# agentmorris/MegaDetector

Hardware: AMD Instinct MI355X
Metric: images/sec (whole node) MDv5a @1280px batch inference (higher is better)
Workload: dtype bf16

## Files before the change

include/mdhip.h:

```cpp
#ifndef MDHIP_H
#define MDHIP_H

#include <stddef.h>
#include <stdint.h>

#include "mdjpeg.h"

#ifdef __cplusplus
extern "C" {
#endif

#define MDHIP_OK            0
#define MDHIP_EINVAL       -1
#define MDHIP_EHIP         -2
#define MDHIP_ENOMEM       -3
#define MDHIP_EUNSUPPORTED -4
#define MDHIP_ECAPACITY    -5

#define MDHIP_DTYPE_BF16 0
#define MDHIP_DTYPE_FP8  1
#define MDHIP_DTYPE_FP16 2

#define MDHIP_CONV      0
#define MDHIP_C3        1
// ... 198 lines not shown
int mdhip_read_op_tensor(mdhip_ctx* ctx, int op, int which, int n, float* out, int* c, int* h, int* w, void* hip_stream);
int mdhip_read_op_weights(mdhip_ctx* ctx, int op, float* w, float* b, int* c_out, int* c_in, int* kh, int* kw);

int mdhip_dwconv3x3_on(mdhip_ctx* ctx, const uint16_t* in, int ld_in, const float* weight, const float* bias, const uint16_t* res,
                       uint16_t* out, int n, int h, int w, int c, int grp, int grp_stride, int grp_off, int act, void* hip_stream);
int mdhip_attention_on(mdhip_ctx* ctx, const uint16_t* qkv, uint16_t* out, int n, int n_tokens, int heads, void* hip_stream);
int mdhip_dfl_decode_on(mdhip_ctx* ctx, const float* box, const float* cls, int nc, int n, int ny, int nx, float stride, float* pred,
                        void* hip_stream);

int mdhip_adown_pool_on(mdhip_ctx* ctx, const uint16_t* in, uint16_t* a, uint16_t* b, int n, int h, int w, int c_in,
                        void* hip_stream);
int mdhip_cbfuse_on(mdhip_ctx* ctx, const uint16_t* const* src, const int32_t* factor, int n_src, const uint16_t* last,
                    uint16_t* out, int n, int h, int w, int c, void* hip_stream);

typedef struct {
    char    name[48];
    int32_t kind;
    int32_t layer;
    int32_t m, n, k;
    double  flops;
    double  bytes;
    int32_t cfg;
    int32_t ntaps, stride, has_res;
} mdhip_op_info;

long long mdhip_plan_describe(const mdhip_model* model, int dtype, int max_batch, int max_h, int max_w, char* buf, size_t cap);
int mdhip_num_ops(mdhip_ctx* ctx);
int mdhip_get_op_info(mdhip_ctx* ctx, int op, mdhip_op_info* out);
int mdhip_forward_timed(mdhip_ctx* ctx, int n, int h, int w, float* ms, void* hip_stream);
int mdhip_time_forwards(mdhip_ctx* ctx, int enable);
int mdhip_forward_times(mdhip_ctx* ctx, float* ms, int max_n);
int mdhip_set_op_cfg(mdhip_ctx* ctx, int op, int cfg);
int mdhip_num_conv_cfgs(void);
int mdhip_op_supports_cfg(mdhip_ctx* ctx, int op, int cfg);
int mdhip_cfg_is_bitwise(int cfg);
const char* mdhip_conv_cfg_name(int cfg);
typedef struct {
    int32_t m, n, k;
    int32_t ntaps, stride;
    int32_t has_res;
    int32_t cfg;
    int32_t batch;
} mdhip_tuned;
int mdhip_set_tuned(mdhip_ctx* ctx, const mdhip_tuned* entries, int n);
int mdhip_set_fuse(mdhip_ctx* ctx, int on);
int mdhip_set_graph(mdhip_ctx* ctx, int mode, int max_n);
int mdhip_set_option(mdhip_ctx* ctx, const char* name, int value);
int mdhip_time_op(mdhip_ctx* ctx, int op, int n, int h, int w, int iters, float* ms_avg,
                  void* hip_stream);
#define MDHIP_LAUNCHES_NO_FUSE 1
#define MDHIP_LAUNCHES_NO_FUSE_DECODE 2
#define MDHIP_LAUNCHES_NO_PAIR 4
#define MDHIP_LAUNCHES_ISOLATED 8
#define MDHIP_LAUNCHES_CALIBRATING 16
#define MDHIP_LAUNCHES_AUGMENTED 32
#define MDHIP_LAUNCHES_AFTER_OTHERS 64
long long mdhip_launches_describe(const mdhip_model* model, int dtype, int max_batch, int max_h, int max_w, const mdhip_tuned* tuned,
                                  int n_tuned, int n, int h, int w, unsigned flags, const int32_t* forced, int n_forced, char* buf,
                                  size_t cap);

const char* mdhip_version(void);

#ifdef __cplusplus
}
#endif
#endif
```

megadetector_amd/_lib.py:

```python

import ctypes as C
import os

import numpy as np

from .jpeg_host import mdjpeg_change_options

_HERE = os.path.dirname(os.path.abspath(__file__))
LIB_PATH = os.path.join(_HERE, 'libmdhip.so')

MDHIP_OK = 0
MDHIP_EINVAL = -1
MDHIP_ECAPACITY = -5
MDHIP_EUNSUPPORTED = -4
MDHIP_DTYPE_BF16 = 0
MDHIP_DTYPE_FP8 = 1
MDHIP_DTYPE_FP16 = 2
MDHIP_LAUNCHES_NO_FUSE, MDHIP_LAUNCHES_NO_FUSE_DECODE, MDHIP_LAUNCHES_NO_PAIR, MDHIP_LAUNCHES_ISOLATED = 1, 2, 4, 8
MDHIP_LAUNCHES_CALIBRATING, MDHIP_LAUNCHES_AUGMENTED, MDHIP_LAUNCHES_AFTER_OTHERS = 16, 32, 64


class mdhip_conv(C.Structure):
    _fields_ = [('weight', C.POINTER(C.c_float)), ('bias', C.POINTER(C.c_float)),
                ('c_out', C.c_int32), ('c_in', C.c_int32), ('kh', C.c_int32), ('kw', C.c_int32)]


class mdhip_layer(C.Structure):
    _fields_ = [('type', C.c_int32), ('n_from', C.c_int32), ('from_', C.c_int32 * 4),
                ('c_out', C.c_int32), ('k', C.c_int32), ('s', C.c_int32), ('p', C.c_int32),
                ('n', C.c_int32), ('shortcut', C.c_int32), ('first_conv', C.c_int32)]


class mdhip_model(C.Structure):
    _fields_ = [('n_layers', C.c_int32), ('layers', C.POINTER(mdhip_layer)),
                ('n_convs', C.c_int32), ('convs', C.POINTER(mdhip_conv)),
                ('nc', C.c_int32), ('na', C.c_int32), ('nl', C.c_int32),
                ('anchors_px', C.POINTER(C.c_float)), ('strides', C.POINTER(C.c_float))]


class mdhip_letterbox(C.Structure):
    _fields_ = [('src_h', C.c_int32), ('src_w', C.c_int32), ('resized_h', C.c_int32),
                ('resized_w', C.c_int32), ('top', C.c_int32), ('left', C.c_int32), ('interp', C.c_int32)]
# ... 16 lines not shown
class mdhip_classifier_crop(C.Structure):
    _fields_ = [('src', C.c_void_p), ('pitch', C.c_int64), ('src_w', C.c_int32), ('src_h', C.c_int32),
                ('canvas_w', C.c_int32), ('canvas_h', C.c_int32), ('off_x', C.c_int32), ('off_y', C.c_int32)]


class mdhip_thumbnail(C.Structure):
    _fields_ = [('src', C.c_void_p), ('pitch', C.c_int64), ('src_w', C.c_int32), ('src_h', C.c_int32),
                ('canvas_w', C.c_int32), ('canvas_h', C.c_int32), ('off_x', C.c_int32), ('off_y', C.c_int32),
                ('out_w', C.c_int32), ('out_h', C.c_int32), ('dst', C.c_void_p), ('dst_pitch', C.c_int64)]


class mdhip_rde_box(C.Structure):
    _fields_ = [('x', C.c_double), ('y', C.c_double), ('w', C.c_double), ('h', C.c_double),
                ('group', C.c_int32), ('category', C.c_int32)]


mdhip_change_options = mdjpeg_change_options


class mdhip_op_info(C.Structure):
    _fields_ = [('name', C.c_char * 48), ('kind', C.c_int32), ('layer', C.c_int32),
                ('m', C.c_int32), ('n', C.c_int32), ('k', C.c_int32),
                ('flops', C.c_double), ('bytes', C.c_double), ('cfg', C.c_int32),
                ('ntaps', C.c_int32), ('stride', C.c_int32), ('has_res', C.c_int32)]


class mdhip_tuned(C.Structure):
    _fields_ = [('m', C.c_int32), ('n', C.c_int32), ('k', C.c_int32), ('ntaps', C.c_int32),
                ('stride', C.c_int32), ('has_res', C.c_int32), ('cfg', C.c_int32), ('batch', C.c_int32)]


_P = C.c_void_p
SYMBOLS = {
    'mdhip_create': (C.c_int, [C.POINTER(mdhip_model), C.c_int, C.c_int, C.c_int, C.c_int, C.c_int, C.POINTER(_P)]),
    'mdhip_create_images': (C.c_int, [C.c_int, C.POINTER(_P)]),
    'mdhip_destroy': (None, [_P]),
    'mdhip_last_error': (C.c_char_p, [_P]),
    'mdhip_preprocess': (C.c_int, [_P, C.POINTER(_P), C.POINTER(mdhip_letterbox), C.c_int, C.c_int, C.c_int, _P]),
    'mdhip_preprocess_windows': (C.c_int, [_P, C.POINTER(_P), C.POINTER(mdhip_letterbox), C.POINTER(C.c_int64),
                                           C.POINTER(C.c_int64), C.c_int, C.c_int, C.c_int, _P]),
    'mdhip_forward': (C.c_int, [_P, C.c_int, C.c_int, C.c_int, _P]),
    'mdhip_jpeg_reconstruct': (C.c_int, [_P, C.POINTER(mdhip_jpeg_image), C.c_int, C.POINTER(_P), _P]),
    'mdhip_jpeg_entropy_decode': (C.c_int, [_P, C.POINTER(mdhip_jpeg_scan), C.c_int, C.c_int, C.POINTER(C.c_int32), _P]),
    'mdhip_jpeg_entropy_stats': (C.c_int, [_P, C.POINTER(C.c_int64)]),
    'mdhip_jpeg_recompress': (C.c_int, [_P, C.POINTER(_P), C.POINTER(C.c_int32), C.POINTER(C.c_int32), C.POINTER(C.c_int64),
                                        C.c_int, C.POINTER(C.c_uint16), C.POINTER(C.c_uint16), C.POINTER(_P), _P]),
    'mdhip_jpeg_encode': (C.c_int, [_P, C.POINTER(_P), C.POINTER(C.c_int32), C.POINTER(C.c_int32), C.POINTER(C.c_int64), C.c_int,
# ... 109 lines not shown
```

megadetector_amd/csrc/conv_v2.cpp:

```cpp

#include <algorithm>
#include <type_traits>

#include "conv_device.h"

namespace mdhip {
namespace MDHIP_ST {

namespace {

constexpr int v2_lds_bytes(int bm, int bn) { return 2 * (bm + bn) * 128; }
constexpr int v2_ring_lds_bytes(int bm, int bn) { return (3 * bm + 2 * bn) * 128; }
constexpr int v2_blocks_per_cu(int bm, int bn, int nw) {
    int b = 163840 / v2_lds_bytes(bm, bn);
    if (b > 32 / nw) b = 32 / nw;
    if (b > 2) b = 2;
    return b < 1 ? 1 : b;
}
constexpr int v2_waves_per_simd(int bm, int bn, int nw) {
    int w = v2_blocks_per_cu(bm, bn, nw) * nw / 4;
    return w < 1 ? 1 : w;
}

}
// ... 459 lines not shown
        advance();
        if constexpr (RA == 3) {
            lb_advance();
            ca = ca == 2 ? 0 : ca + 1;
        }
        stamp(4);
        if (++c_kt == KT) {
            epilogue(c_tile);
            c_kt = 0;
            c_tile += tile_step;
        }
        stamp(5);
    }
    if constexpr ((PROF & 1) != 0) {
        if (lane == 0 && p.dbg) {
            unsigned long long* d = (unsigned long long*)p.dbg + ((size_t)blockIdx.x * NW + wave) * 8;
            for (int k = 0; k < 6; ++k) d[k] = t_acc[k];
            d[6] = (unsigned long long)total_steps;
            d[7] = (unsigned long long)__builtin_amdgcn_s_getreg(((4 - 1) << 11) | (0 << 6) | 20) ;
        }
    }
#endif
}

#define MDHIP_CONV2_CFGS(X) \
    X(0, 160, 160, 2, 2)    \
    X(1, 128, 160, 2, 2)    \
    X(2, 160, 80, 2, 1)     \
    X(3, 128, 80, 4, 1)     \
    X(4, 96, 160, 2, 2)     \
    X(5, 64, 160, 1, 2)     \
    X(6, 192, 160, 4, 2)    \
    X(7, 256, 160, 4, 2)    \
    X(8, 320, 160, 4, 2)
#define MDHIP_CONV2_RING(X) \
    X(9, 96, 160, 2, 2)     \
    X(10, 64, 160, 1, 2)    \
    X(11, 320, 160, 4, 2)   \
    X(12, 256, 160, 4, 2)
#define MDHIP_CONV2_DEC(X) \
    X(0, 160, 160, 2, 2)   \
    X(2, 160, 80, 2, 1)    \
    X(3, 128, 80, 4, 1)    \
    X(8, 320, 160, 4, 2)
#define MDHIP_CONV2_PROF(X) \
    X(13, 160, 160, 2, 2, 1)  \
// ... 13 lines not shown
    {bm, bn, (wm) * (wn) * 64, (size_t)v2_lds_bytes(bm, bn), v2_blocks_per_cu(bm, bn, (wm) * (wn)), \
     "v2:" #bm "x" #bn "/" #wm "x" #wn},
    MDHIP_CONV2_CFGS(X)
#undef X
#define X(id, bm, bn, wm, wn)                                                                        \
    {bm, bn, (wm) * (wn) * 64, (size_t)v2_ring_lds_bytes(bm, bn), 163840 / v2_ring_lds_bytes(bm, bn) >= 2 ? 2 : 1, "v2:" #bm "x" #bn "/" #wm "x" #wn "/a3"},
    MDHIP_CONV2_RING(X)
#undef X
#define X(id, bm, bn, wm, wn, prof)                                                                  \
    {bm, bn, (wm) * (wn) * 64, (size_t)v2_lds_bytes(bm, bn), v2_blocks_per_cu(bm, bn, (wm) * (wn)), \
     "v2prof" #prof ":" #bm "x" #bn "/" #wm "x" #wn},
    MDHIP_CONV2_PROF(X)
#undef X
#define X(id, bm, bn, wm, wn, prof)                                                                  \
    {bm, bn, (wm) * (wn) * 64, (size_t)v2_ring_lds_bytes(bm, bn), 1, "v2prof" #prof ":" #bm "x" #bn "/" #wm "x" #wn "/a3"},
    MDHIP_CONV2_PROFRING(X)
#undef X
};
constexpr int kNumPlain2 = 0 MDHIP_CONV2_CFGS(MDHIP_COUNT_ROW);
constexpr int kNumCfgs2 = kNumPlain2 MDHIP_CONV2_RING(MDHIP_COUNT_ROW);
constexpr int kNumProf = 0 MDHIP_CONV2_PROF(MDHIP_COUNT_ROW) MDHIP_CONV2_PROFRING(MDHIP_COUNT_ROW);

namespace {
enum { V2_PLAIN = 0, V2_PW1, V2_PW2, V2_UP, V2_DEV, V2_DEV_PW };
ConvInstTable conv2_insts() {
    static const ConvInst t[] = {
#define X(id, bm, bn, wm, wn)                                                                                         \
    MDHIP_INST(id, V2_PLAIN, (wm) * (wn) * 64, v2_lds_bytes(bm, bn), conv_v2_kernel<bm, bn, wm, wn>)                  \
    MDHIP_INST(id, V2_PW1, (wm) * (wn) * 64, v2_lds_bytes(bm, bn), conv_v2_kernel<bm, bn, wm, wn, 0, false, 1>)       \
    MDHIP_INST(id, V2_PW2, (wm) * (wn) * 64, v2_lds_bytes(bm, bn), conv_v2_kernel<bm, bn, wm, wn, 0, false, 2>)
        MDHIP_CONV2_CFGS(X)
#undef X
#define X(id, bm, bn, wm, wn)                                                                                         \
    MDHIP_INST(id, V2_PW1, (wm) * (wn) * 64, v2_ring_lds_bytes(bm, bn), conv_v2_kernel<bm, bn, wm, wn, 0, false, 1, 3>) \
    MDHIP_INST(id, V2_PW2, (wm) * (wn) * 64, v2_ring_lds_bytes(bm, bn), conv_v2_kernel<bm, bn, wm, wn, 0, false, 2, 3>)
        MDHIP_CONV2_RING(X)
#undef X
#define X(id, bm, bn, wm, wn, prof) MDHIP_INST(id, V2_DEV, (wm) * (wn) * 64, v2_lds_bytes(bm, bn), conv_v2_kernel<bm, bn, wm, wn, prof>)
        MDHIP_CONV2_PROF(X)
#undef X
#define X(id, bm, bn, wm, wn, prof) MDHIP_INST(id, V2_DEV_PW, (wm) * (wn) * 64, v2_ring_lds_bytes(bm, bn), conv_v2_kernel<bm, bn, wm, wn, prof, false, 1, 3>)
        MDHIP_CONV2_PROFRING(X)
#undef X
#define X(id, bm, bn, wm, wn) MDHIP_INST(id, CONV_KEY_DEC, (wm) * (wn) * 64, v2_lds_bytes(bm, bn), conv_v2_kernel<bm, bn, wm, wn, 0, false, 1, 2, 1>)
        MDHIP_CONV2_DEC(X)
#undef X
        MDHIP_INST(0, V2_UP, 256, v2_lds_bytes(160, 160), conv_v2_kernel<160, 160, 2, 2, 0, true>)
    };
    return {t, (int)(sizeof(t) / sizeof(t[0]))};
}
const ConvInst* conv2_pick(int cfg, const ConvArgs& a) {
    const ConvInstTable t = conv2_insts();
    if (a.in_up) return a.dec_pred ? nullptr : conv_find_inst(t, cfg, V2_UP);
    const bool pw = a.ntaps == 1 && a.stride == 1 && a.pad == 0 && a.H == a.Ho && a.W == a.Wo, whole = (a.C8 & 7) == 0;
    if (a.dec_pred) return pw && whole && a.out_f32 ? conv_find_inst(t, cfg, CONV_KEY_DEC) : nullptr;
    if (cfg >= kNumCfgs2) {
        const ConvInst* dev = conv_find_inst(t, cfg, V2_DEV);
        return dev || !(pw && whole) ? dev : conv_find_inst(t, cfg, V2_DEV_PW);
    }
    return conv_find_inst(t, cfg, !pw ? V2_PLAIN : whole ? V2_PW1 : V2_PW2);
}

bool conv2_cfg_is_ring(int cfg) { return cfg >= kNumPlain2 && cfg < kNumCfgs2; }
bool conv2_shape_ok(const ConvArgs& a) {
    if (a.in_up && !(a.ntaps == 1 && a.stride == 1 && (a.H % 2) == 0 && (a.W % 2) == 0 && a.up_slabs > 0 &&
                     a.up_slabs * 8 <= a.C8 && !a.in_f8))
        return false;
    return a.C8 >= 8 && a.kw <= 3 && a.ntaps <= 9 && (a.k_pad % 64) == 0;
}
bool conv2_supports(int cfg, const ConvArgs& a) {
    if (cfg < 0 || cfg >= kNumCfgs2 + kNumProf) return false;
    if (conv2_cfg_is_ring(cfg) && a.k_pad < 3 * 64) return false;
    return conv2_shape_ok(a) && conv2_pick(cfg, a) != nullptr;
}

hipError_t conv2_launch(int cfg, const ConvArgs& a, hipStream_t s) {
    if (cfg < 0 || cfg >= kNumCfgs2 + kNumProf || !conv2_shape_ok(a)) return hipErrorInvalidValue;
    ConvArgs p = a;
    conv_set_rcp(p);
    const dim3 grid = conv_tile_grid(p, g_cfgs2[cfg]);
    return conv_launch_inst(conv2_pick(cfg, a), grid, p, s);
}
}

MDHIP_CONV_FAMILY(conv_v2, CONV_V2, g_cfgs2, kNumCfgs2, kNumProf, true, false, true, conv2_supports, conv2_launch, conv2_insts)

}
}
```

megadetector_amd/csrc/mdhip_capi.cpp:

```cpp

#include <algorithm>
#include <climits>
#include <cmath>
#include <cstdarg>
#include <cstdio>
#include <cstdlib>
#include <cstring>

#include "mdhip_ctx.h"

static thread_local std::string g_create_error;

int mdhip::fail(mdhip_ctx* ctx, int code, const char* fmt, ...) {
    char buf[512];
    va_list ap;
    va_start(ap, fmt);
    vsnprintf(buf, sizeof(buf), fmt, ap);
    va_end(ap);
    if (ctx) ctx->err = buf; else g_create_error = buf;
    return code;
}

int mdhip::check_shape(mdhip_ctx* ctx, int n, int h, int w) {
    if (n < 1 || n > ctx->max_batch) return fail(ctx, MDHIP_EINVAL, "batch %d outside [1,%d]", n, ctx->max_batch);
// ... 213 lines not shown
    return (long long)text.size();
}

long long mdhip_launches_describe(const mdhip_model* model, int dtype, int max_batch, int max_h, int max_w, const mdhip_tuned* tuned,
                                  int n_tuned, int n, int h, int w, unsigned flags, const int32_t* forced, int n_forced, char* buf,
                                  size_t cap) {
    if (int rc = check_create_args(model, dtype, max_batch, max_h, max_w)) return rc;
    if (n_tuned < 0 || (n_tuned > 0 && !tuned) || n_forced < 0 || (n_forced > 0 && !forced))
        return fail(nullptr, MDHIP_EINVAL, "mdhip_launches_describe: bad table or forced list");
    mdhip_ctx ctx;
    ctx.pair_enabled = !(flags & MDHIP_LAUNCHES_NO_PAIR);
    PlannedWeights pw;
    std::string err;
    if (int rc = plan_context(&ctx, model, dtype, max_batch, max_h, max_w, &pw, &err)) return fail(nullptr, rc, "%s", err.c_str());
    ctx.arena = (char*)(uintptr_t)(1ull << 40);
    ctx.warena = (char*)(uintptr_t)(2ull << 40);
    int rc = check_shape(&ctx, n, h, w);
    if (!rc) rc = mdhip_set_tuned(&ctx, tuned, n_tuned);
    for (int i = 0; i < n_forced && !rc; ++i) rc = mdhip_set_op_cfg(&ctx, forced[2 * i], forced[2 * i + 1]);
    if (rc) return fail(nullptr, rc, "%s", ctx.err.empty() ? "mdhip_launches_describe: bad forced list" : ctx.err.c_str());
    const bool fuse = !(flags & MDHIP_LAUNCHES_NO_FUSE), fuse_decode = !(flags & MDHIP_LAUNCHES_NO_FUSE_DECODE);
    (void)mdhip_set_fuse(&ctx, fuse);
    (void)mdhip_set_option(&ctx, "fuse_decode", fuse_decode);
    auto resolve_as = [&](unsigned kind, int rn, int rh, int rw) {
        Pass pass(&ctx, nullptr, num_anchors_for(&ctx, rh, rw), (kind & MDHIP_LAUNCHES_ISOLATED) != 0, (kind & MDHIP_LAUNCHES_CALIBRATING) != 0);
        if (kind & MDHIP_LAUNCHES_AUGMENTED) ctx.cur_tta.scale = 0.83f;
        return resolved_for(&ctx, rn, rh, rw);
    };
    if (flags & MDHIP_LAUNCHES_AFTER_OTHERS)
        for (int round = 0; round < 4; ++round) {
            (void)mdhip_set_fuse(&ctx, round == 1 ? !fuse : fuse);
            (void)mdhip_set_option(&ctx, "fuse_decode", round == 2 ? !fuse_decode : fuse_decode);
            for (unsigned kind : {0u, (unsigned)MDHIP_LAUNCHES_ISOLATED, (unsigned)MDHIP_LAUNCHES_CALIBRATING, (unsigned)MDHIP_LAUNCHES_AUGMENTED}) {
                (void)resolve_as(kind, n, h, w);
                (void)resolve_as(kind, 1, ctx.max_stride * 2, ctx.max_stride * 3);
            }
        }
    const std::string text = describe_launches(&ctx, *resolve_as(flags, n, h, w));
    if (buf && cap) snprintf(buf, cap, "%s", text.c_str());
    return (long long)text.size();
}

void mdhip_destroy(mdhip_ctx* ctx) {
    if (!ctx) return;
    (void)hipSetDevice(ctx->device);
    drop_graphs(ctx);
// ... 516 lines not shown
                    w[(((size_t)oc * CI + ci) * KH + r) * KW + q] = st_to_f32(p[k], f16);
                }
    return MDHIP_OK;
}

int mdhip_num_ops(mdhip_ctx* ctx) { return ctx ? (int)ctx->ops.size() : MDHIP_EINVAL; }

int mdhip_get_op_info(mdhip_ctx* ctx, int op, mdhip_op_info* out) {
    NEED_MODEL(ctx);
    if (!ctx || !out || op < 0 || op >= (int)ctx->ops.size()) return MDHIP_EINVAL;
    const Op& o = ctx->ops[op];
    memset(out, 0, sizeof(*out));
    snprintf(out->name, sizeof(out->name), "%s", o.name.c_str());
    out->kind = o.kind == OP_DFL ? OP_DECODE : o.kind;
    if (o.kind == OP_ADOWN || o.kind == OP_CBFUSE) out->kind = o.kind - 1;
    out->layer = o.layer;
    const Launch L = ctx->last_ran ? ctx->last_ran->ops[op] : Launch();
    out->m = L.gm;
    out->n = L.gn;
    out->k = L.gk;
    out->flops = L.flops;
    out->bytes = L.bytes;
    out->cfg = L.how == RUN_IN_FRONT ? -2 : (o.kind == OP_CONV && L.how == RUN_LAUNCH) ? L.cfg : -1;
    if (o.kind == OP_CONV || o.kind == OP_DW) {
        const PackedConv& pc = ctx->packed[o.pc];
        out->ntaps = pc.kh * pc.kw;
        out->stride = o.stride;
        out->has_res = o.has_res ? 1 : 0;
    }
    return MDHIP_OK;
}

int mdhip_num_conv_cfgs(void) { return conv_num_cfgs(); }

int mdhip_op_supports_cfg(mdhip_ctx* ctx, int op, int cfg) {
    NEED_MODEL(ctx);
    if (!ctx || op < 0 || op >= (int)ctx->ops.size()) return MDHIP_EINVAL;
    if (ctx->ops[op].kind != OP_CONV || cfg < 0 || cfg >= conv_num_cfgs()) return 0;
    ConvArgs a{};
    const int h = ctx->last_h ? ctx->last_h : ctx->max_stride, w = ctx->last_w ? ctx->last_w : ctx->max_stride;
    conv_args(ctx, ctx->ops[op], ctx->last_n ? ctx->last_n : 1, h, w, a);
    return conv_api(ctx).supports(cfg, a) ? 1 : 0;
}

const char* mdhip_conv_cfg_name(int cfg) { return (cfg >= 0 && cfg < conv_num_cfgs()) ? conv_cfg(cfg).name : ""; }

// ... 2 lines not shown
int mdhip_set_tuned(mdhip_ctx* ctx, const mdhip_tuned* entries, int n) {
    NEED_MODEL(ctx);
    if (!ctx || n < 0 || (n > 0 && !entries)) return MDHIP_EINVAL;
    for (int i = 0; i < n; ++i)
        if (entries[i].cfg < 0 || entries[i].cfg >= conv_num_cfgs())
            return fail(ctx, MDHIP_EINVAL, "tuned entry %d: cfg %d outside [0,%d)", i, entries[i].cfg, conv_num_cfgs());
    ctx->tuned.assign(entries, entries + n);
    launches_changed(ctx);
    return MDHIP_OK;
}

int mdhip_set_fuse(mdhip_ctx* ctx, int on) {
    NEED_MODEL(ctx);
    ctx->fuse_enabled = on != 0;
    launches_changed(ctx);
    return MDHIP_OK;
}

int mdhip_set_option(mdhip_ctx* ctx, const char* name, int value) {
    NEED_MODEL(ctx);
    if (!ctx || !name) return MDHIP_EINVAL;
    if (!strcmp(name, "letterbox_general")) ctx->letterbox_general = value != 0;
    else if (!strcmp(name, "fuse_decode")) ctx->fuse_decode = value != 0;
    else return fail(ctx, MDHIP_EINVAL, "unknown option '%s'", name);
    launches_changed(ctx);
    return MDHIP_OK;
}

int mdhip_set_graph(mdhip_ctx* ctx, int mode, int max_n) {
    NEED_MODEL(ctx);
    if (!ctx || mode < 0 || mode > 2) return MDHIP_EINVAL;
    ctx->graph_mode = mode;
    if (max_n > 0) ctx->graph_max_n = max_n;
    if (mode == 0) drop_graphs(ctx);
    return MDHIP_OK;
}

int mdhip_set_op_cfg(mdhip_ctx* ctx, int op, int cfg) {
    NEED_MODEL(ctx);
    if (!ctx || op < 0 || op >= (int)ctx->ops.size()) return MDHIP_EINVAL;
    if (ctx->ops[op].kind != OP_CONV) return fail(ctx, MDHIP_EINVAL, "op %d is not a conv", op);
    if (cfg < -1 || cfg >= conv_num_cfgs()) return fail(ctx, MDHIP_EINVAL, "cfg %d outside [-1,%d)", cfg, conv_num_cfgs());
    ctx->ops[op].forced_cfg = cfg;
    launches_changed(ctx);
    return MDHIP_OK;
}
// ... 3 lines not shown
```

megadetector_amd/csrc/mdhip_ctx.h:

```cpp
#pragma once

#include <map>
#include <memory>
#include <string>
#include <tuple>
#include <vector>

#include "../../include/mdhip.h"
#include "mdhip_internal.h"

using namespace mdhip;

namespace mdhip {

int fail(mdhip_ctx* ctx, int code, const char* fmt, ...);

#define HIP_TRY(ctx, expr)                                                                   \
    do {                                                                                     \
        hipError_t e__ = (expr);                                                             \
        if (e__ != hipSuccess)                                                               \
            return fail(ctx, MDHIP_EHIP, "%s failed: %s (%s:%d)", #expr, hipGetErrorString(e__), \
                        __FILE__, __LINE__);                                                 \
    } while (0)

// ... 160 lines not shown
    NmsScratch nms_scr{};
    size_t nms_kv_off[6] = {}, nms_seg_off = 0;
    size_t nms_out_off = 0, nms_cnt_off = 0;
    size_t geom_off = 0;
    DevBuffer stage;
    DevBuffer jpeg_planes;
    DevBuffer jpeg_entropy;
    DevBuffer jpeg_encode;
    DevBuffer blur;
    DevBuffer resample;
    DevBuffer draw;
    DevBuffer classify;
    DevBuffer change;
    long long jpeg_entropy_stats[4] = {0, 0, 0, 0};
    int last_n = 0, last_h = 0, last_w = 0;
    int step_n = 0, step_h = 0, step_w = 0;
    std::string err;
    bool calibrated = false, calibrating = false;
    int n_f8 = 0;
    std::vector<std::vector<int>> fuse_groups;
    bool fuse_enabled = true, fuse_suspended = false;
    bool pair_enabled = true;
    bool fuse_decode = true;
    bool letterbox_general = false;
    std::vector<hipEvent_t> events;
    std::vector<mdhip_tuned> tuned;
    static constexpr int kFwdRing = 64;
    bool time_forward = false;
    hipEvent_t fwd_ev[kFwdRing][2] = {};
    long long fwd_count = 0;
    uint8_t* geom_host = nullptr;
    int geom_slot = 0;
    hipEvent_t geom_ev[4] = {nullptr, nullptr, nullptr, nullptr};
    float* nms_host_out[MDHIP_NMS_SLOTS] = {};
    int32_t* nms_host_cnt[MDHIP_NMS_SLOTS] = {};
    hipEvent_t nms_ev[MDHIP_NMS_SLOTS] = {};
    int nms_slot_n[MDHIP_NMS_SLOTS] = {};
    int graph_mode = 0;
    int graph_max_n = 8;
    hipStream_t capture_stream = nullptr;
    struct GraphSlot { hipGraphExec_t exec = nullptr; int seen = 0; bool disabled = false; long long last_use = 0; };
    std::map<std::tuple<int, int, int, int>, GraphSlot> graphs;
    static constexpr int kMaxGraphs = 32;
    long long graph_clock = 0;
    std::map<std::tuple<int, int, int, int>, std::shared_ptr<Resolved>> resolved;
    static constexpr int kMaxResolved = 64;
// ... 9 lines not shown
```

megadetector_amd/csrc/mdhip_exec.cpp:

```cpp

#include <algorithm>
#include <cmath>
#include <cstring>

#include "mdhip_ctx.h"

namespace mdhip {

const ConvRegistry& conv_api(const mdhip_ctx* ctx) { return ctx->dtype == MDHIP_DTYPE_FP16 ? st_f16::conv_registry : st_bf16::conv_registry; }
int conv_num_cfgs() { return st_bf16::conv_registry.num_cfgs(); }
const ConvCfg& conv_cfg(int i) { return st_bf16::conv_registry.cfg(i); }
bool conv_cfg_is_bitwise_family(int c) { return st_bf16::conv_registry.is_bitwise_family(c); }

int choose_cfg(int M, int n_rows) {
    const ConvFamily& v1 = *st_bf16::conv_registry.fam[CONV_IGEMM];
    int best = 0;
    float best_score = -1.f;
    for (int i = 0; i < v1.n_cfgs; ++i) {
        const ConvCfg& c = v1.cfgs[i];
        const int tn = (n_rows + c.bn - 1) / c.bn, tm = (M + c.bm - 1) / c.bm;
        const float useful = ((float)n_rows / (tn * c.bn)) * ((float)M / ((float)tm * c.bm));
        const float fill = std::min(1.0f, (float)tm * tn / 512.0f);
        const float score = useful * (0.35f + 0.65f * fill) * c.prior;
        if (score > best_score) { best_score = score; best = i; }
// ... 38 lines not shown
    a.k_pad = pc.k_pad;
    a.ntaps = pc.kh * pc.kw;
    a.kw = pc.kw;
    a.stride = op.stride;
    a.pad = op.pad;
    a.act = op.act;
    a.out_f32 = op.out_f32;
    if (op.out_f32) {
        a.out = ctx->arena + op.f32_off;
        a.ld_out = op.f32_ld;
    } else {
        a.out = ctx->arena + op.out.off;
        a.ld_out = op.out.ld;
    }
    a.res = op.has_res ? (const uint16_t*)(ctx->arena + op.res.off) : nullptr;
    a.ld_res = op.has_res ? op.res.ld : 0;
    a.tiles_n = 1;
    a.out_qscale = 1.0f;
    a.wgt4 = pc.w4_off ? (const uint16_t*)(ctx->warena + pc.w4_off) : nullptr;
    a.k_pad4 = pc.k_pad4;
    a.groups = pc.groups;
    a.wgt4p = (pc.w4p_off && ctx->pair_enabled) ? (const uint16_t*)(ctx->warena + pc.w4p_off) : nullptr;
    a.k_pad4p = pc.k_pad4p;
    if (ctx->dtype == MDHIP_DTYPE_FP8 && !ctx->calibrating) {
        if (op.f8_in) {
            a.in_f8 = 1;
            a.wgt8 = (const uint8_t*)(ctx->warena + pc.w8_off);
            a.scale = (const float*)(ctx->warena + pc.scale_off);
            a.k_pad8 = pc.k_pad8;
            a.groups8 = pc.groups8;
            a.C8 = (op.in.c + 15) / 16;
        }
        a.out_f8 = op.f8_out ? 1 : 0;
    }
}

namespace {

void conv_stats(const mdhip_ctx* ctx, const Op& op, const ConvArgs& a, int n, Launch& L) {
    const PackedConv& pc = ctx->packed[op.pc];
    L.gm = a.M;
    L.gn = pc.c_out;
    L.gk = pc.k_real;
    L.flops = 2.0 * (double)a.M * pc.c_out * pc.k_real;
    L.bytes = (double)n * a.H * a.W * op.in.c * 2.0 + (double)a.M * pc.c_out * (op.out_f32 ? 4.0 : 2.0) +
              (double)pc.c_out * pc.k_real * 2.0 + (op.has_res ? (double)a.M * pc.c_out * 2.0 : 0.0);
// ... 323 lines not shown
```

megadetector_amd/csrc/mdhip_internal.h:

```cpp
#pragma once

#include <hip/hip_runtime.h>
#include <stdint.h>

#include <algorithm>

struct MdClassifyCrop;

struct ChgWeights;
struct MdjImage;
struct MdjEncCrop;
struct MdjEncTables;
struct MdjKeepRect;

namespace mdhip {

__host__ __device__ inline uint16_t f32_to_bf16(float f) {
    union { float f; uint32_t u; } v;
    v.f = f;
    uint32_t u = v.u;
    if ((u & 0x7fffffffu) > 0x7f800000u) return (uint16_t)((u >> 16) | 0x40);
    u += 0x7fffu + ((u >> 16) & 1u);
    return (uint16_t)(u >> 16);
}
// ... 77 lines not shown
    int out_f32;
    int tiles_n, tiles_m, tiles_per_xcd, m_streams;
    const uint16_t* wgt4;
    int k_pad4, groups;
    const uint16_t* wgt4p;
    int k_pad4p;
    const uint8_t* wgt8;
    const float*   scale;
    int k_pad8, groups8;
    int in_f8, out_f8;
    float out_qscale;
    void* dbg;
    int dev_param;
    const uint16_t* wgt_pre;
    const float*    bias_pre;
    int k_pad_pre;
    const uint16_t* in_up;
    int ld_up, up_slabs;
    float* dec_pred;
    const float* dec_anchors;
    float dec_stride;
    int dec_level_off, dec_n_anchors;
    unsigned rcp_howo, rcp_wo;
};
inline unsigned conv_rcp32(int d) { return d <= 1 ? 0xffffffffu : (unsigned)(0x100000000ull / (unsigned)d); }
inline void conv_set_rcp(ConvArgs& p) { p.rcp_howo = conv_rcp32(p.HoWo); p.rcp_wo = conv_rcp32(p.Wo); }
#if defined(__HIP_DEVICE_COMPILE__) || defined(__HIPCC__)
__device__ __forceinline__ float mdhip_sigmoid_exact(float x) { return 1.0f / (1.0f + expf(-x)); }
__device__ __forceinline__ void mdhip_decode_box(float l0, float l1, float l2, float l3, int x, int y, float stride, float aw, float ah,
                                                 float& cx, float& cy, float& bw, float& bh) {
#pragma clang fp contract(off)
    const float s0 = mdhip_sigmoid_exact(l0), s1 = mdhip_sigmoid_exact(l1);
    const float s2 = mdhip_sigmoid_exact(l2), s3 = mdhip_sigmoid_exact(l3);
    cx = (s0 * 2.0f + ((float)x - 0.5f)) * stride;
    cy = (s1 * 2.0f + ((float)y - 0.5f)) * stride;
    const float w2 = s2 * 2.0f, h2 = s3 * 2.0f;
    bw = (w2 * w2) * aw;
    bh = (h2 * h2) * ah;
}
#endif

struct ConvCfg {
    int bm, bn, threads;
    size_t lds_bytes;
    int blocks_per_cu;
    const char* name;
// ... 21 lines not shown
constexpr int CONV_KEY_DEC = 100;
#define MDHIP_INST(local, key, threads, lds, ...) {(const void*)(__VA_ARGS__), (local), (key), (threads), (size_t)(lds)},
inline const ConvInst* conv_find_inst(ConvInstTable t, int local, int key) {
    for (int i = 0; i < t.n; ++i)
        if (t.rows[i].local == local && t.rows[i].key == key) return &t.rows[i];
    return nullptr;
}
inline hipError_t conv_launch_inst(const ConvInst* inst, dim3 grid, const ConvArgs& p, hipStream_t s) {
    if (!inst) return hipErrorInvalidValue;
    void* args[] = {(void*)&p};
    return hipLaunchKernel(inst->fn, grid, dim3((unsigned)inst->threads), args, inst->lds_bytes, s);
}

struct ConvFamily {
    ConvFamilyId id;
    const ConvCfg* cfgs;
    int n_cfgs, n_dev;
    bool bitwise;
    bool f8_in;
    bool f8_out;
    bool (*supports)(int local, const ConvArgs& a);
    hipError_t (*launch)(int local, const ConvArgs& a, hipStream_t s);
    ConvInstTable (*insts)();
};
#if defined(__HIP_DEVICE_COMPILE__)
#define MDHIP_CONV_FAMILY(name, ...)
#else
#define MDHIP_CONV_FAMILY(name, ...) extern const ConvFamily name = {__VA_ARGS__};
#endif
inline bool conv_family_takes(const ConvFamily& f, const ConvArgs& a) { return f.f8_in == (a.in_f8 != 0) && (!a.out_f8 || f.f8_out); }
inline bool conv_decode_ok(bool cfg_decodes, const ConvArgs& a) { return !a.dec_pred || (cfg_decodes && a.out_f32 && (a.N % 8) == 0); }
inline bool conv5_shape_ok(const ConvArgs& a, int bm) {
    return a.wgt4 != nullptr && a.ntaps == 9 && a.kw == 3 && a.stride == 1 && a.pad == 1 && a.Ho == a.H && a.Wo == a.W && a.C8 >= 8 &&
           (a.N % 8) == 0 && (long long)(2 * a.W + bm + 16) * a.ld_in * 2 + 4096 < 0x7fffffffLL;
}

struct ConvRegistry {
    const ConvFamily* fam[CONV_NUM_FAMILIES];

    int num_cfgs() const {
        int n = 0;
        for (const ConvFamily* f : fam) n += f->n_cfgs;
        return n;
    }
    const ConvFamily* find(int cfg, int* local) const {
        if (cfg < 0) return nullptr;
// ... 19 lines not shown
        const ConvFamily* f = find(cfg, &l);
        return f ? f->bitwise : true;
    }
    bool cfg_decodes(int cfg) const {
        int l = 0;
        const ConvFamily* f = find(cfg, &l);
        return f && conv_find_inst(f->insts(), l, CONV_KEY_DEC) != nullptr;
    }
    bool supports(int cfg, const ConvArgs& a) const {
        int l = 0;
        const ConvFamily* f = find(cfg, &l);
        return f && (!a.dec_pred || conv_decode_ok(cfg_decodes(cfg), a)) && conv_family_takes(*f, a) && f->supports(l, a);
    }
    bool supports_decoding(int cfg, const ConvArgs& a) const {
        float none = 0.f;
        ConvArgs d = a;
        if (!d.dec_pred) d.dec_pred = &none;
        return supports(cfg, d);
    }
    hipError_t launch(int cfg, const ConvArgs& a, hipStream_t s) const {
        int l = 0;
        const ConvFamily* f = find(cfg, &l);
        return f && conv_family_takes(*f, a) ? f->launch(l, a, s) : hipErrorInvalidValue;
    }
    hipError_t launch_dev(ConvFamilyId family, int k, const ConvArgs& a, hipStream_t s) const {
        const ConvFamily* f = fam[family];
        return k >= 0 && k < f->n_dev ? f->launch(f->n_cfgs + k, a, s) : hipErrorInvalidValue;
    }
    hipError_t init() const {
        hipError_t e = hipSuccess;
        for (const ConvFamily* f : fam) {
            const ConvInstTable t = f->insts();
            for (int i = 0; i < t.n && e == hipSuccess; ++i)
                e = hipFuncSetAttribute(t.rows[i].fn, hipFuncAttributeMaxDynamicSharedMemorySize, (int)t.rows[i].lds_bytes);
        }
        return e;
    }
};
#define MDHIP_CONV_FAMILIES extern const ConvFamily conv_igemm, conv_v2, conv_v5, conv_v5s, conv_v5c, conv_v6, conv_f8, conv_v7; \
                            extern const ConvRegistry conv_registry;
namespace st_bf16 {
MDHIP_CONV_FAMILIES
}
namespace st_f16 {
MDHIP_CONV_FAMILIES
}
// ... 225 lines not shown
```

megadetector_amd/hip_backend.py:

```python

import ctypes as C
import json
import os
from contextlib import contextmanager

import numpy as np

from . import _lib
from ._lib import HipError
from .jpeg_host import quant_tables
from .yolo_model import DETECT_TYPES, MDHIP_CBFUSE, MDHIP_DETECT_DDFL, detect_inputs


_DTYPES = {'bf16': _lib.MDHIP_DTYPE_BF16, 'fp8': _lib.MDHIP_DTYPE_FP8, 'fp16': _lib.MDHIP_DTYPE_FP16}


def model_description(weights):
    keep = []
    specs = weights.specs
    convs = []
    layers = (_lib.mdhip_layer * len(specs))()
    for i, s in enumerate(specs):
        L = layers[i]
        L.type = s.type
# ... 55 lines not shown


def _described(call, what):
    lib = _lib.load()
    need = call(None, 0)
    if need >= 0:
        buf = C.create_string_buffer(need + 1)
        need = call(buf, need + 1)
    if need < 0:
        err = HipError('{} failed ({}): {}'.format(what, need, lib.mdhip_last_error(None).decode()))
        err.code = int(need)
        raise err
    return buf.value.decode()


def describe_plan(weights, dtype='bf16', max_batch=32, max_h=1280, max_w=1280):
    lib = _lib.load()
    m, keep = model_description(weights)
    args = (C.byref(m), _DTYPES[dtype], int(max_batch), int(max_h), int(max_w))
    return _described(lambda buf, cap: lib.mdhip_plan_describe(*args, buf, cap), 'mdhip_plan_describe')


def describe_launches(weights, dtype, capacity, tuned_entries, n, h, w, fuse=True, fuse_decode=True, pair=True, isolated=False,
                      calibrating=False, augmented=False, forced=None, after_others=False):
    lib = _lib.load()
    m, keep = model_description(weights)
    arr, n_tuned = tuned_array(lib, tuned_entries or [])
    flags = ((not fuse) * _lib.MDHIP_LAUNCHES_NO_FUSE | (not fuse_decode) * _lib.MDHIP_LAUNCHES_NO_FUSE_DECODE |
             (not pair) * _lib.MDHIP_LAUNCHES_NO_PAIR | bool(isolated) * _lib.MDHIP_LAUNCHES_ISOLATED |
             bool(calibrating) * _lib.MDHIP_LAUNCHES_CALIBRATING | bool(augmented) * _lib.MDHIP_LAUNCHES_AUGMENTED |
             bool(after_others) * _lib.MDHIP_LAUNCHES_AFTER_OTHERS)
    by_name = {lib.mdhip_conv_cfg_name(i).decode(): i for i in range(lib.mdhip_num_conv_cfgs())}
    pairs = [v for op, cfg in sorted((forced or {}).items()) for v in (int(op), by_name[cfg] if isinstance(cfg, str) else int(cfg))]
    farr = (C.c_int32 * max(1, len(pairs)))(*pairs)
    args = (C.byref(m), _DTYPES[dtype], *[int(v) for v in capacity], arr, n_tuned, int(n), int(h), int(w), flags, farr, len(pairs) // 2)
    return _described(lambda buf, cap: lib.mdhip_launches_describe(*args, buf, cap), 'mdhip_launches_describe')


def table_entries(dtype='bf16'):
    path = HipContext.TUNED_PATH
    alt = path.replace('.json', '_{}.json'.format(dtype))
    if dtype != 'bf16' and os.path.exists(alt):
        path = alt
    return json.load(open(path)).get('entries', [])


def _window_arrays(ptrs, sizes, pitches):
    n = len(ptrs)
    return (C.cast((C.c_void_p * n)(*[int(v) for v in ptrs]), C.POINTER(C.c_void_p)), (C.c_int32 * n)(*[int(v[0]) for v in sizes]),
            (C.c_int32 * n)(*[int(v[1]) for v in sizes]), (C.c_int64 * n)(*[int(v) for v in pitches]))


def _quant_array(quants, n):
    packed = np.zeros((max(n, 1), 2, 64), dtype=np.uint16)
# ... 420 lines not shown
        out = np.empty((n, c.value, h.value, w.value), dtype=np.float32)
        self._check(self.lib.mdhip_read_op_tensor(self.h, int(op), int(which), int(n), _lib.np_ptr(out), *args), 'mdhip_read_op_tensor')
        return out

    def read_op_weights(self, op):
        dims = [C.c_int() for _ in range(4)]
        refs = [C.byref(d) for d in dims]
        self._check(self.lib.mdhip_read_op_weights(self.h, int(op), None, None, *refs), 'mdhip_read_op_weights')
        w = np.empty(tuple(d.value for d in dims), dtype=np.float32)
        b = np.empty((dims[0].value,), dtype=np.float32)
        self._check(self.lib.mdhip_read_op_weights(self.h, int(op), _lib.np_ptr(w), _lib.np_ptr(b), *refs), 'mdhip_read_op_weights')
        return w, b

    def num_ops(self):
        return self.lib.mdhip_num_ops(self.h)

    def op_infos(self):
        res = []
        for i in range(self.num_ops()):
            info = _lib.mdhip_op_info()
            self._check(self.lib.mdhip_get_op_info(self.h, i, C.byref(info)), 'mdhip_get_op_info')
            res.append(dict(op=i, name=info.name.decode(), kind=info.kind, layer=info.layer, m=info.m,
                            n=info.n, k=info.k, flops=info.flops, bytes=info.bytes, cfg=info.cfg,
                            ntaps=info.ntaps, stride=info.stride, has_res=info.has_res))
        return res

    def forward_timed(self, n, h, w, stream=0):
        ms = np.zeros((self.num_ops(),), dtype=np.float32)
        self._check(self.lib.mdhip_forward_timed(self.h, n, h, w, _lib.np_ptr(ms), C.c_void_p(stream)),
                    'mdhip_forward_timed')
        return ms

    def time_forwards(self, enable=True):
        self._check(self.lib.mdhip_time_forwards(self.h, 1 if enable else 0), 'mdhip_time_forwards')

    def forward_times(self, max_n=64):
        ms = np.zeros((max_n,), dtype=np.float32)
        n = self.lib.mdhip_forward_times(self.h, _lib.np_ptr(ms), int(max_n))
        if n < 0:
            self._check(n, 'mdhip_forward_times')
        return ms[:n].copy()

    def set_op_cfg(self, op, cfg):
        self._check(self.lib.mdhip_set_op_cfg(self.h, op, cfg), 'mdhip_set_op_cfg')

    def set_fuse(self, on):
        self._check(self.lib.mdhip_set_fuse(self.h, 1 if on else 0), 'mdhip_set_fuse')
# ... 25 lines not shown
```

Before: 1101.

## Add weight-stationary streaming kernel for large 160-channel pointwise convs

Result: faster. 1115 (median of 6 runs) (+1.2%).

```diff
diff --git a/include/mdhip.h b/include/mdhip.h
--- a/include/mdhip.h
+++ b/include/mdhip.h
@@ -244,6 +244,7 @@
     double  bytes;
     int32_t cfg;
     int32_t ntaps, stride, has_res;
+    int32_t variant;
 } mdhip_op_info;
 
 long long mdhip_plan_describe(const mdhip_model* model, int dtype, int max_batch, int max_h, int max_w, char* buf, size_t cap);
@@ -276,6 +277,7 @@
 #define MDHIP_LAUNCHES_ISOLATED 8
 #define MDHIP_LAUNCHES_CALIBRATING 16
 #define MDHIP_LAUNCHES_AUGMENTED 32
+#define MDHIP_LAUNCHES_NO_PW_STREAM 128
 #define MDHIP_LAUNCHES_AFTER_OTHERS 64
 long long mdhip_launches_describe(const mdhip_model* model, int dtype, int max_batch, int max_h, int max_w, const mdhip_tuned* tuned,
                                   int n_tuned, int n, int h, int w, unsigned flags, const int32_t* forced, int n_forced, char* buf,
diff --git a/megadetector_amd/_lib.py b/megadetector_amd/_lib.py
--- a/megadetector_amd/_lib.py
+++ b/megadetector_amd/_lib.py
@@ -17,7 +17,7 @@
 MDHIP_DTYPE_FP8 = 1
 MDHIP_DTYPE_FP16 = 2
 MDHIP_LAUNCHES_NO_FUSE, MDHIP_LAUNCHES_NO_FUSE_DECODE, MDHIP_LAUNCHES_NO_PAIR, MDHIP_LAUNCHES_ISOLATED = 1, 2, 4, 8
-MDHIP_LAUNCHES_CALIBRATING, MDHIP_LAUNCHES_AUGMENTED, MDHIP_LAUNCHES_AFTER_OTHERS = 16, 32, 64
+MDHIP_LAUNCHES_CALIBRATING, MDHIP_LAUNCHES_AUGMENTED, MDHIP_LAUNCHES_AFTER_OTHERS, MDHIP_LAUNCHES_NO_PW_STREAM = 16, 32, 64, 128
 
 
 class mdhip_conv(C.Structure):
@@ -80,7 +80,7 @@
     _fields_ = [('name', C.c_char * 48), ('kind', C.c_int32), ('layer', C.c_int32),
                 ('m', C.c_int32), ('n', C.c_int32), ('k', C.c_int32),
                 ('flops', C.c_double), ('bytes', C.c_double), ('cfg', C.c_int32),
-                ('ntaps', C.c_int32), ('stride', C.c_int32), ('has_res', C.c_int32)]
+                ('ntaps', C.c_int32), ('stride', C.c_int32), ('has_res', C.c_int32), ('variant', C.c_int32)]
 
 
 class mdhip_tuned(C.Structure):
diff --git a/megadetector_amd/csrc/conv_v2.cpp b/megadetector_amd/csrc/conv_v2.cpp
--- a/megadetector_amd/csrc/conv_v2.cpp
+++ b/megadetector_amd/csrc/conv_v2.cpp
@@ -505,6 +505,8 @@
     }
 #endif
 }
+
+#include "conv_v2_stream.h"
 
 #define MDHIP_CONV2_CFGS(X) \
     X(0, 160, 160, 2, 2)    \
@@ -564,7 +566,8 @@
 constexpr int kNumProf = 0 MDHIP_CONV2_PROF(MDHIP_COUNT_ROW) MDHIP_CONV2_PROFRING(MDHIP_COUNT_ROW);
 
 namespace {
-enum { V2_PLAIN = 0, V2_PW1, V2_PW2, V2_UP, V2_DEV, V2_DEV_PW };
+enum { V2_PLAIN = 0, V2_PW1, V2_PW2, V2_UP, V2_DEV, V2_DEV_PW, V2_STREAM };
+constexpr int kStreamMinM = 307200;
 ConvInstTable conv2_insts() {
     static const ConvInst t[] = {
 #define X(id, bm, bn, wm, wn)                                                                                         \
@@ -588,8 +591,21 @@
         MDHIP_CONV2_DEC(X)
 #undef X
         MDHIP_INST(0, V2_UP, 256, v2_lds_bytes(160, 160), conv_v2_kernel<160, 160, 2, 2, 0, true>)
+        MDHIP_INST(0, V2_STREAM, 256, 0, conv_v2_stream_kernel)
     };
     return {t, (int)(sizeof(t) / sizeof(t[0]))};
+}
+bool conv2_streams(const ConvArgs& a, bool pw) {
+    if (a.pw_stream <= 0 || (a.pw_stream == 1 && a.M < kStreamMinM) || !pw || a.k_pad != 192 || a.C8 != 20 || a.n_rows != 160 || a.N != 160 ||
+        a.act != 1 || a.out_f32 || a.res || a.in_up || a.in_f8 || a.out_f8 || a.dec_pred || a.M <= 0 || (a.ld_in % 8) != 0 ||
+        (a.ld_out % 8) != 0 || a.ld_in < 160 || a.ld_out < 160 || ((uintptr_t)a.in % 16) != 0 || ((uintptr_t)a.out % 16) != 0)
+        return false;
+    const long long in0 = (long long)(uintptr_t)a.in, out0 = (long long)(uintptr_t)a.out;
+    const long long in1 = in0 + ((long long)(a.M - 1) * a.ld_in + 160) * 2, out1 = out0 + ((long long)(a.M - 1) * a.ld_out + 160) * 2;
+    if (in1 <= out0 || out1 <= in0) return true;
+    if (a.ld_in != a.ld_out) return false;
+    const long long pitch = (long long)a.ld_in * 2, r = (((out0 - in0) % pitch) + pitch) % pitch;
+    return r >= 320 && r + 320 <= pitch;
 }
 const ConvInst* conv2_pick(int cfg, const ConvArgs& a) {
     const ConvInstTable t = conv2_insts();
@@ -600,6 +616,7 @@
         const ConvInst* dev = conv_find_inst(t, cfg, V2_DEV);
         return dev || !(pw && whole) ? dev : conv_find_inst(t, cfg, V2_DEV_PW);
     }
+    if (cfg >= 0 && conv2_streams(a, pw)) return conv_find_inst(t, 0, V2_STREAM);
     return conv_find_inst(t, cfg, !pw ? V2_PLAIN : whole ? V2_PW1 : V2_PW2);
 }
 
@@ -620,12 +637,22 @@
     if (cfg < 0 || cfg >= kNumCfgs2 + kNumProf || !conv2_shape_ok(a)) return hipErrorInvalidValue;
     ConvArgs p = a;
     conv_set_rcp(p);
-    const dim3 grid = conv_tile_grid(p, g_cfgs2[cfg]);
-    return conv_launch_inst(conv2_pick(cfg, a), grid, p, s);
-}
-}
-
-MDHIP_CONV_FAMILY(conv_v2, CONV_V2, g_cfgs2, kNumCfgs2, kNumProf, true, false, true, conv2_supports, conv2_launch, conv2_insts)
-
-}
-}
+    dim3 grid = conv_tile_grid(p, g_cfgs2[cfg]);
+    const ConvInst* inst = conv2_pick(cfg, a);
+    if (inst && inst->key == V2_STREAM) {
+        const int streams = std::max(1, std::min(1024, (p.M + 15) / 16 / 2));
+        grid = dim3((unsigned)((streams + 3) / 4));
+    }
+    return conv_launch_inst(inst, grid, p, s);
+}
+int conv2_variant(int cfg, const ConvArgs& a) {
+    if (cfg < 0 || cfg >= kNumCfgs2 + kNumProf || !conv2_shape_ok(a)) return -1;
+    const ConvInst* inst = conv2_pick(cfg, a);
+    return inst ? inst->key : -1;
+}
+}
+
+MDHIP_CONV_FAMILY(conv_v2, CONV_V2, g_cfgs2, kNumCfgs2, kNumProf, true, false, true, conv2_supports, conv2_launch, conv2_insts, conv2_variant)
+
+}
+}
diff --git a/megadetector_amd/csrc/conv_v2_stream.h b/megadetector_amd/csrc/conv_v2_stream.h
--- /dev/null
+++ b/megadetector_amd/csrc/conv_v2_stream.h
@@ -0,0 +1,82 @@
+#pragma once
+
+__global__ void __launch_bounds__(256, 1)
+conv_v2_stream_kernel(const ConvArgs p) {
+#if defined(__HIP_DEVICE_COMPILE__)
+    constexpr int NC = 10;
+    constexpr int D = 3;
+    constexpr int KS = 6, KS_REAL = 5;
+    const int lane = threadIdx.x & 63;
+    const int wave = __builtin_amdgcn_readfirstlane(threadIdx.x >> 6);
+    const int px = lane & 15, q = lane >> 4;
+    const int stream = (int)(blockIdx.x * 4) + wave;
+    const int n_streams = (int)(gridDim.x * 4);
+    const int n_groups = (p.M + 15) >> 4;
+    const int iters = (n_groups + n_streams - 1) / n_streams;
+
+    const __amdgpu_buffer_rsrc_t w_rsrc = __builtin_amdgcn_make_buffer_rsrc((void*)p.wgt, 0, p.n_rows * p.k_pad * 2, kRsrcFlags);
+    const __amdgpu_buffer_rsrc_t b_rsrc = __builtin_amdgcn_make_buffer_rsrc((void*)p.bias, 0, p.n_rows * 4, kRsrcFlags);
+    frag8_t w[NC][KS];
+    f32x4 bv[NC];
+#pragma unroll
+    for (int j = 0; j < NC; ++j) {
+        const unsigned row = (unsigned)((j * 16 + px) * p.k_pad + q * 8) * 2u;
+#pragma unroll
+        for (int s = 0; s < KS; ++s)
+            w[j][s] = __builtin_bit_cast(frag8_t, __builtin_amdgcn_raw_buffer_load_b128(w_rsrc, (int)row + s * 64, 0, 0));
+        bv[j] = __builtin_bit_cast(f32x4, __builtin_amdgcn_raw_buffer_load_b128(b_rsrc, (j * 16 + q * 4) * 4, 0, 0));
+    }
+    frag8_t xz = __builtin_bit_cast(frag8_t, u32x4{0u, 0u, 0u, 0u});
+    asm volatile("" : "+v"(xz));
+
+    const unsigned x_off = (unsigned)(px * p.ld_in * 2 + q * 16);
+    const unsigned o_pair = (unsigned)(px * p.ld_out + q * 8) * 2u;
+    auto group_of = [&](int it) __attribute__((always_inline)) { return it * n_streams + stream; };
+    auto rows_rsrc = [&](const void* base, int ld, int grp) __attribute__((always_inline)) {
+        const long long left = ((long long)p.M - (long long)grp * 16) * ld * 2;
+        return __builtin_amdgcn_make_buffer_rsrc((void*)((const uint16_t*)base + (long long)grp * 16 * ld), 0,
+                                                 (int)(left <= 0 ? 0LL : left > 0x7fffffffLL ? 0x7fffffffLL : left), kRsrcFlags);
+    };
+    u32x4 x[D][KS_REAL];
+    auto load = [&](int slot, int it) __attribute__((always_inline)) {
+        const __amdgpu_buffer_rsrc_t r = rows_rsrc(p.in, p.ld_in, group_of(it));
+#pragma unroll
+        for (int s = 0; s < KS_REAL; ++s) x[slot][s] = __builtin_amdgcn_raw_buffer_load_b128(r, (int)x_off + s * 64, 0, 0);
+    };
+    auto compute = [&](int slot, int it) __attribute__((always_inline)) {
+#pragma clang fp contract(off)
+        f32x4 acc[NC];
+#pragma unroll
+        for (int j = 0; j < NC; ++j) acc[j] = f32x4{0.f, 0.f, 0.f, 0.f};
+#pragma unroll
+        for (int s = 0; s < KS; ++s)
+#pragma unroll
+            for (int j = 0; j < NC; ++j)
+                acc[j] = MDHIP_MFMA(w[j][s], s < KS_REAL ? __builtin_bit_cast(frag8_t, x[slot][s]) : xz, acc[j]);
+        const __amdgpu_buffer_rsrc_t o_rsrc = rows_rsrc(p.out, p.ld_out, group_of(it));
+        float v[NC][4];
+#pragma unroll
+        for (int j = 0; j < NC; ++j) {
+            mdhip_bias4(acc[j], bv[j], v[j]);
+            mdhip_silu4(v[j]);
+        }
+#pragma unroll
+        for (int j = 0; j + 1 < NC; j += 2)
+            __builtin_amdgcn_raw_buffer_store_b128(conv_pack_pair(v[j], v[j + 1]), o_rsrc, (int)(o_pair + (unsigned)(j * 32)), 0, 0);
+    };
+#pragma unroll
+    for (int d = 0; d < D - 1; ++d) {
+        load(d, d);
+        MDHIP_FENCE();
+    }
+    for (int it = 0; it < iters; it += D) {
+#pragma unroll
+        for (int d = 0; d < D; ++d) {
+            load((d + D - 1) % D, it + d + D - 1);
+            MDHIP_FENCE();
+            compute(d, it + d);
+            MDHIP_FENCE();
+        }
+    }
+#endif
+}
diff --git a/megadetector_amd/csrc/mdhip_capi.cpp b/megadetector_amd/csrc/mdhip_capi.cpp
--- a/megadetector_amd/csrc/mdhip_capi.cpp
+++ b/megadetector_amd/csrc/mdhip_capi.cpp
@@ -259,6 +259,7 @@
     const bool fuse = !(flags & MDHIP_LAUNCHES_NO_FUSE), fuse_decode = !(flags & MDHIP_LAUNCHES_NO_FUSE_DECODE);
     (void)mdhip_set_fuse(&ctx, fuse);
     (void)mdhip_set_option(&ctx, "fuse_decode", fuse_decode);
+    (void)mdhip_set_option(&ctx, "pw_stream", !(flags & MDHIP_LAUNCHES_NO_PW_STREAM));
     auto resolve_as = [&](unsigned kind, int rn, int rh, int rw) {
         Pass pass(&ctx, nullptr, num_anchors_for(&ctx, rh, rw), (kind & MDHIP_LAUNCHES_ISOLATED) != 0, (kind & MDHIP_LAUNCHES_CALIBRATING) != 0);
         if (kind & MDHIP_LAUNCHES_AUGMENTED) ctx.cur_tta.scale = 0.83f;
@@ -821,6 +822,13 @@
     out->flops = L.flops;
     out->bytes = L.bytes;
     out->cfg = L.how == RUN_IN_FRONT ? -2 : (o.kind == OP_CONV && L.how == RUN_LAUNCH) ? L.cfg : -1;
+    out->variant = -1;
+    if (o.kind == OP_CONV && L.how == RUN_LAUNCH) {
+        ConvArgs a = L.a;
+        float none = 0.f;
+        a.dec_pred = L.decodes ? &none : nullptr;
+        out->variant = conv_api(ctx).variant(L.cfg, a);
+    }
     if (o.kind == OP_CONV || o.kind == OP_DW) {
         const PackedConv& pc = ctx->packed[o.pc];
         out->ntaps = pc.kh * pc.kw;
@@ -869,6 +877,7 @@
     if (!ctx || !name) return MDHIP_EINVAL;
     if (!strcmp(name, "letterbox_general")) ctx->letterbox_general = value != 0;
     else if (!strcmp(name, "fuse_decode")) ctx->fuse_decode = value != 0;
+    else if (!strcmp(name, "pw_stream")) ctx->pw_stream = value <= 0 ? 0 : value >= 2 ? 2 : 1;
     else return fail(ctx, MDHIP_EINVAL, "unknown option '%s'", name);
     launches_changed(ctx);
     return MDHIP_OK;
diff --git a/megadetector_amd/csrc/mdhip_ctx.h b/megadetector_amd/csrc/mdhip_ctx.h
--- a/megadetector_amd/csrc/mdhip_ctx.h
+++ b/megadetector_amd/csrc/mdhip_ctx.h
@@ -206,6 +206,7 @@
     bool fuse_enabled = true, fuse_suspended = false;
     bool pair_enabled = true;
     bool fuse_decode = true;
+    int pw_stream = 1;
     bool letterbox_general = false;
     std::vector<hipEvent_t> events;
     std::vector<mdhip_tuned> tuned;
diff --git a/megadetector_amd/csrc/mdhip_exec.cpp b/megadetector_amd/csrc/mdhip_exec.cpp
--- a/megadetector_amd/csrc/mdhip_exec.cpp
+++ b/megadetector_amd/csrc/mdhip_exec.cpp
@@ -84,6 +84,7 @@
     a.groups = pc.groups;
     a.wgt4p = (pc.w4p_off && ctx->pair_enabled) ? (const uint16_t*)(ctx->warena + pc.w4p_off) : nullptr;
     a.k_pad4p = pc.k_pad4p;
+    a.pw_stream = ctx->pw_stream;
     if (ctx->dtype == MDHIP_DTYPE_FP8 && !ctx->calibrating) {
         if (op.f8_in) {
             a.in_f8 = 1;
diff --git a/megadetector_amd/csrc/mdhip_internal.h b/megadetector_amd/csrc/mdhip_internal.h
--- a/megadetector_amd/csrc/mdhip_internal.h
+++ b/megadetector_amd/csrc/mdhip_internal.h
@@ -123,6 +123,7 @@
     float dec_stride;
     int dec_level_off, dec_n_anchors;
     unsigned rcp_howo, rcp_wo;
+    int pw_stream;
 };
 inline unsigned conv_rcp32(int d) { return d <= 1 ? 0xffffffffu : (unsigned)(0x100000000ull / (unsigned)d); }
 inline void conv_set_rcp(ConvArgs& p) { p.rcp_howo = conv_rcp32(p.HoWo); p.rcp_wo = conv_rcp32(p.Wo); }
@@ -190,6 +191,7 @@
     bool (*supports)(int local, const ConvArgs& a);
     hipError_t (*launch)(int local, const ConvArgs& a, hipStream_t s);
     ConvInstTable (*insts)();
+    int (*variant)(int local, const ConvArgs& a);
 };
 #if defined(__HIP_DEVICE_COMPILE__)
 #define MDHIP_CONV_FAMILY(name, ...)
@@ -255,6 +257,11 @@
         int l = 0;
         const ConvFamily* f = find(cfg, &l);
         return f && conv_family_takes(*f, a) ? f->launch(l, a, s) : hipErrorInvalidValue;
+    }
+    int variant(int cfg, const ConvArgs& a) const {
+        int l = 0;
+        const ConvFamily* f = find(cfg, &l);
+        return f && f->variant && conv_family_takes(*f, a) ? f->variant(l, a) : -1;
     }
     hipError_t launch_dev(ConvFamilyId family, int k, const ConvArgs& a, hipStream_t s) const {
         const ConvFamily* f = fam[family];
diff --git a/megadetector_amd/hip_backend.py b/megadetector_amd/hip_backend.py
--- a/megadetector_amd/hip_backend.py
+++ b/megadetector_amd/hip_backend.py
@@ -101,14 +101,14 @@
 
 
 def describe_launches(weights, dtype, capacity, tuned_entries, n, h, w, fuse=True, fuse_decode=True, pair=True, isolated=False,
-                      calibrating=False, augmented=False, forced=None, after_others=False):
+                      calibrating=False, augmented=False, forced=None, after_others=False, pw_stream=True):
     lib = _lib.load()
     m, keep = model_description(weights)
     arr, n_tuned = tuned_array(lib, tuned_entries or [])
     flags = ((not fuse) * _lib.MDHIP_LAUNCHES_NO_FUSE | (not fuse_decode) * _lib.MDHIP_LAUNCHES_NO_FUSE_DECODE |
              (not pair) * _lib.MDHIP_LAUNCHES_NO_PAIR | bool(isolated) * _lib.MDHIP_LAUNCHES_ISOLATED |
              bool(calibrating) * _lib.MDHIP_LAUNCHES_CALIBRATING | bool(augmented) * _lib.MDHIP_LAUNCHES_AUGMENTED |
-             bool(after_others) * _lib.MDHIP_LAUNCHES_AFTER_OTHERS)
+             bool(after_others) * _lib.MDHIP_LAUNCHES_AFTER_OTHERS | (not pw_stream) * _lib.MDHIP_LAUNCHES_NO_PW_STREAM)
     by_name = {lib.mdhip_conv_cfg_name(i).decode(): i for i in range(lib.mdhip_num_conv_cfgs())}
     pairs = [v for op, cfg in sorted((forced or {}).items()) for v in (int(op), by_name[cfg] if isinstance(cfg, str) else int(cfg))]
     farr = (C.c_int32 * max(1, len(pairs)))(*pairs)
@@ -575,7 +575,7 @@
             self._check(self.lib.mdhip_get_op_info(self.h, i, C.byref(info)), 'mdhip_get_op_info')
             res.append(dict(op=i, name=info.name.decode(), kind=info.kind, layer=info.layer, m=info.m,
                             n=info.n, k=info.k, flops=info.flops, bytes=info.bytes, cfg=info.cfg,
-                            ntaps=info.ntaps, stride=info.stride, has_res=info.has_res))
+                            ntaps=info.ntaps, stride=info.stride, has_res=info.has_res, variant=info.variant))
         return res
 
     def forward_timed(self, n, h, w, stream=0):
```
